# erererq/gym-lorenz

Hardware: NVIDIA B200
Metric: env_steps_per_sec (higher is better)
Workload: dtype f64

## Files before the change

### gym_lorenz_b200/csrc/chaos_b200.cu

```cuda
#include <math.h>
#include <pthread.h>
#include <sched.h>
#include <stdarg.h>
#include <time.h>
#include <stdio.h>
#include <stdlib.h>
#include <string.h>

#include "kernels_common.cuh"
#include "host_copy.h"

cudaError_t cl_launch_derivatives(int kind, const void* state, const float* action, void* out,
                                  int64_t n, cudaStream_t st);

using cl::KParams;

struct CopyHelper;

namespace {

const cl_layout kLayouts[CL_ENV_KIND_COUNT] = {
     {8, 4, 0, 6, 3, 0, -500.0, 500.0, -HUGE_VAL, HUGE_VAL, 0, 0},
     {8, 10, 0, 6, 3, 0, -500.0, 500.0, -HUGE_VAL, HUGE_VAL, 0, 0},
     {8, 9, 0, 8, 3, 0, -2.0, 2.0, -HUGE_VAL, HUGE_VAL, 0, 0},
// ... 355 lines not shown
  const double eff = (double)W / (double)(((W + nsched - 1) / nsched) * nsched);
  return eff < 0.95;
}

extern "C" int cl_rollout(cl_ctx* ctx, void* stream, const cl_buffers* buf, const cl_io* io,
                          const cl_rollout_desc* d) {
  if (!ctx) return fail(nullptr, CL_EINVAL, "null ctx");
  if (!io || !d || d->T < 1) return fail(ctx, CL_EINVAL, "cl_rollout: io/desc required, T >= 1");
  if (io->noise) return fail(ctx, CL_EINVAL, "cl_rollout: noise override is single-step only");
  KParams p;
  int r = fill_params(ctx, buf, io, p);
  if (r) return r;
  p.T = d->T; p.act_ts = d->act_ts; p.obs_ts = d->obs_ts; p.rew_ts = d->rew_ts; p.done_ts = d->done_ts;
  p.synth_amp = (float)d->synth_amp;
  cudaStream_t st = (cudaStream_t)stream;
  CU(cudaSetDevice(ctx->cfg.device));
  int chunk = CL_DYN_CHUNK_DEFAULT;
  if (const char* ov = getenv("CHAOS_B200_DYN_CHUNK")) { const int c = atoi(ov); if (c >= 1 && c <= 16) chunk = c; }
  int mode = cl::MODE_ROLLOUT;
  alignas(64) CUtensorMap tmap;
  if (want_dynamic(ctx, d->T, chunk)) {
    const int64_t W = (ctx->cfg.num_envs + 31) / 32;
    if (!ctx->dyn_bps) {
      int occ = 0;
      cudaError_t e = is_parity(ctx->cfg.kind) ? cl_dyn_occupancy_parity(ctx->cfg.kind, chunk, &occ)
                                               : cl_dyn_occupancy_northstar(ctx->cfg.kind, chunk, &occ);
      if (e != cudaSuccess) return fail(ctx, CL_ECUDA, "dyn occupancy query: %s", cudaGetErrorString(e));
      int bps = (int)(W / ((int64_t)ctx->sm_count * 4));
      bps = bps < 1 ? 1 : (bps > 4 ? 4 : bps);
      if (const char* ov = getenv("CHAOS_B200_DYN_BPS")) { const int b = atoi(ov); if (b >= 1 && b <= 16) bps = b; }
      ctx->dyn_bps = occ < bps ? occ : bps;
    }
    if (ctx->dyn_bps >= 1) {
      CU(cudaMemsetAsync(ctx->d_dyn, 0, sizeof(uint32_t) * (size_t)(W + 1), st));
      p.dyn_counter = ctx->d_dyn;
      p.dyn_progress = ctx->d_dyn + 1;
      p.dyn_chunk = chunk;
      p.dyn_nchunks = (d->T + chunk - 1) / chunk;
      p.dyn_nwarps = (int32_t)W;
      const int64_t workers = (int64_t)ctx->sm_count * ctx->dyn_bps;
      const int64_t tasks = W * (int64_t)((d->T + chunk - 1) / chunk);
      p.dyn_grid = (int32_t)(workers * 4 < tasks ? workers : (tasks + 3) / 4);
      p.dyn_tma = (io->action != nullptr && io->act_es == 1 && (io->act_cs % 4) == 0 && (d->act_ts % 4) == 0 &&
                   ((uintptr_t)io->action % 16) == 0 && io->act_cs >= W * 32) ? 1 : 0;
      {
        const char* ov = getenv("CHAOS_B200_SM");
        if (!(ov && ov[0] == '0') && p.dyn_tma) {
          const int grid = (int)(W < ctx->sm_count ? W : ctx->sm_count);
          const int qn = (int)(W / grid), cmax = (int)((W + grid - 1) / grid);
          int workers = qn >= 4 ? 4 * (qn / 4) : qn;
          workers = workers > 16 ? 16 : workers;
          if (workers == 16 && qn < 20) workers = 12;
          if (const char* w = getenv("CHAOS_B200_SM_WORKERS")) { const int k = atoi(w); if (k >= 1 && k <= 16) workers = k < qn ? k : qn; }
          int sc = 16;
          const size_t per_warp = (size_t)ctx->lay.n_state * 32u * (size_t)ctx->lay.real_bytes + 32u * 12u + 28u;
          while (sc > 1 && (size_t)cmax * (2u * (size_t)sc * (size_t)ctx->lay.act_dim * 128u + per_warp) + 256u > 200u * 1024u) sc /= 2;
          if (const char* w = getenv("CHAOS_B200_SM_CHUNK")) { const int k = atoi(w); if (k >= 1 && k <= 16) sc = k; }
          if (sc > d->T) sc = d->T;
          if (cmax <= 64) {
            p.sm_grid = grid; p.sm_workers = workers; p.sm_chunk = sc;
            p.sm_gdiv = 1;
            if (const char* w = getenv("CHAOS_B200_SM_GDIV")) { const int k = atoi(w); if (k >= 1 && k <= 16) p.sm_gdiv = k; }
            p.host_tmap = &tmap;
            p.sm_tmap_ok = action_tensor_map(&tmap, io->action, (uint64_t)W * 32, (uint64_t)ctx->lay.act_dim,
                                             (uint64_t)d->T, (uint64_t)io->act_cs, (uint64_t)d->act_ts, (uint32_t)sc) ? 1 : 0;
            const char* tm = getenv("CHAOS_B200_SM_TMAP");
            if (tm && tm[0] == '0') p.sm_tmap_ok = 0;
// ... 495 lines not shown
```

### gym_lorenz_b200/csrc/envs_northstar.cuh

```cuda
#pragma once
#include "kernels_common.cuh"

namespace cl {

template <typename R>
struct LorenzPar { R sigma, rho, beta; };

template <typename R>
__device__ __forceinline__ void lorenz_rhs_u(const LorenzPar<R>& q, R x, R y, R z, R u1, R u2, R u3,
                                             R& dx, R& dy, R& dz) {
  dx = fma(q.sigma, y - x, u1);
  dy = fma(x, q.rho - z, u2 - y);
  dz = fma(x, y, fma(-q.beta, z, u3));
}

template <typename R>
__device__ __forceinline__ void lorenz_rhs_s(const R sigma, const R beta, R x, R y, R zs, R u1, R u2, R c3,
                                             R& dx, R& dy, R& dz) {
  dx = fma(sigma, y - x, u1);
  dy = fma(-x, zs, u2 - y);
  dz = fma(x, y, fma(-beta, zs, c3));
}

#define CL_LORENZ_RK4_SUBSTEP()                                                                     \
  {                                                                                                 \
    R k1x, k1y, k1z, kx, ky, kz, ax, ay, az;                                                        \
    lorenz_rhs_s(sigma, beta, x, y, zs, u1, u2, c3, k1x, k1y, k1z);                                 \
    ax = fma(h6, k1x, x); ay = fma(h6, k1y, y); az = fma(h6, k1z, zs);                              \
    lorenz_rhs_s(sigma, beta, fma(hh, k1x, x), fma(hh, k1y, y), fma(hh, k1z, zs), u1, u2, c3, kx, ky, kz);   \
    ax = fma(h3, kx, ax); ay = fma(h3, ky, ay); az = fma(h3, kz, az);                               \
    lorenz_rhs_s(sigma, beta, fma(hh, kx, x), fma(hh, ky, y), fma(hh, kz, zs), u1, u2, c3, k1x, k1y, k1z);   \
    ax = fma(h3, k1x, ax); ay = fma(h3, k1y, ay); az = fma(h3, k1z, az);                            \
    lorenz_rhs_s(sigma, beta, fma(h, k1x, x), fma(h, k1y, y), fma(h, k1z, zs), u1, u2, c3, kx, ky, kz);      \
    x = fma(h6, kx, ax); y = fma(h6, ky, ay); zs = fma(h6, kz, az);                                 \
  }

template <typename R>
__device__ __forceinline__ void lorenz_rk4(const R sigma, const R rho, const R beta, const R br, R& x, R& y, R& z,
                                           R u1, R u2, R u3, const R h, const R hh, const R h3, const R h6,
                                           int substeps) {
  R zs = z - rho;
  const R c3 = u3 - br;
#pragma unroll 2
  for (int k = 0; k < substeps; ++k) CL_LORENZ_RK4_SUBSTEP()
  z = zs + rho;
}

template <typename R, int S>
__device__ __forceinline__ void lorenz_rk4_fixed(const R sigma, const R rho, const R beta, const R br, R& x, R& y,
                                                 R& z, R u1, R u2, R u3, const R h, const R hh, const R h3,
                                                 const R h6) {
  R zs = z - rho;
  const R c3 = u3 - br;
#pragma unroll
  for (int k = 0; k < S; ++k) CL_LORENZ_RK4_SUBSTEP()
  z = zs + rho;
}

template <typename R>
__device__ __forceinline__ void lorenz_rk4_any(const R sigma, const R rho, const R beta, const R br, R& x, R& y,
                                               R& z, R u1, R u2, R u3, const R h, const R hh, const R h3,
                                               const R h6, int S) {
  if (S == 16) {
    lorenz_rk4_fixed<R, 16>(sigma, rho, beta, br, x, y, z, u1, u2, u3, h, hh, h3, h6);
    return;
  }
  switch (S) {
    case 8: lorenz_rk4_fixed<R, 8>(sigma, rho, beta, br, x, y, z, u1, u2, u3, h, hh, h3, h6); break;
    case 4: lorenz_rk4_fixed<R, 4>(sigma, rho, beta, br, x, y, z, u1, u2, u3, h, hh, h3, h6); break;
    case 1: lorenz_rk4_fixed<R, 1>(sigma, rho, beta, br, x, y, z, u1, u2, u3, h, hh, h3, h6); break;
    default: lorenz_rk4<R>(sigma, rho, beta, br, x, y, z, u1, u2, u3, h, hh, h3, h6, S); break;
  }
}

template <typename R>
struct EnvLorenzRK4 {
  typedef R real;
  enum { NSTATE = 6, NINT = 0, OBS = 6, ACT = 3, NOISE = 0 };
  struct S { R x, y, z; LorenzPar<R> q; bool uni; };
  __device__ static void load(S& s, const KParams& p, int64_t i) {
    s.x = ldp<R>(p, 0, i); s.y = ldp<R>(p, 1, i); s.z = ldp<R>(p, 2, i);
    s.q.sigma = ldp<R>(p, 3, i); s.q.rho = ldp<R>(p, 4, i); s.q.beta = ldp<R>(p, 5, i);
  }
  __device__ static void prepare(S& s, const KParams& p, bool live) {
    const bool same = !live || (sizeof(R) == 8
        ? (s.q.sigma == (R)p.nom[0] && s.q.rho == (R)p.nom[1] && s.q.beta == (R)p.nom[2])
        : (s.q.sigma == (R)p.nomf[0] && s.q.rho == (R)p.nomf[1] && s.q.beta == (R)p.nomf[2]));
    s.uni = __all_sync(0xffffffffu, same);
  }
// ... 3 lines not shown
  }
  __device__ static void load_sm(S& s, const R* b, unsigned lane) {
    s.x = b[lane]; s.y = b[32 + lane]; s.z = b[64 + lane];
    s.q.sigma = b[96 + lane]; s.q.rho = b[128 + lane]; s.q.beta = b[160 + lane];
  }
  __device__ static void store_sm(const S& s, R* b, unsigned lane) {
    b[lane] = s.x; b[32 + lane] = s.y; b[64 + lane] = s.z;
  }
  __device__ static bool uses_noise(const KParams&) { return false; }
  __device__ static bool finite(const S& s) { return isfinite(s.x + s.y + s.z); }
  __device__ static bool time_limit(const KParams& p, int32_t n) {
    return p.max_steps > 0 && n >= p.max_steps;
  }
  __device__ static void init_persistent(S& s, const KParams& p, const Stream& rng) {
    double j[3] = {1.0, 1.0, 1.0};
    if (p.param_jitter > 0.0) draw_uniform<3>(rng, TAG_PARAM, 1.0 - p.param_jitter, 1.0 + p.param_jitter, j);
    s.q.sigma = (R)(10.0 * j[0]); s.q.rho = (R)(28.0 * j[1]); s.q.beta = (R)((8.0 / 3.0) * j[2]);
    s.x = s.y = s.z = R(0);
  }
  __device__ static void observe(const S& s, R* obs) {
    obs[0] = s.x; obs[1] = s.y; obs[2] = s.z;
    lorenz_rhs_u(s.q, s.x, s.y, s.z, R(0), R(0), R(0), obs[3], obs[4], obs[5]);
  }
  __device__ static void reset(S& s, const KParams&, const Stream& rng, R* obs) {
    double u[3];
    draw_uniform<3>(rng, TAG_RESET, -30.0, 30.0, u);
    s.x = (R)u[0]; s.y = (R)u[1]; s.z = (R)u[2];
    observe(s, obs);
  }
  __device__ static int spec(const S& s, const KParams& p) {
    return (s.uni && p.substeps == 16) ? 1 : 0;
  }
  template <int SPEC>
  __device__ static void step_spec(S& s, const KParams& p, const float* a, const double*, R* obs, R& rew,
                                   bool& term) {
    static_assert(SPEC == 1, "unknown specialisation");
    const float lim = p.act_limit_f;
    const R g = sizeof(R) == 8 ? (R)p.act_gain : (R)p.act_gain_f;
    const R u1 = mul_keep((R)clipf(a[0], -lim, lim), g);
    const R u2 = mul_keep((R)clipf(a[1], -lim, lim), g);
    const R u3 = mul_keep((R)clipf(a[2], -lim, lim), g);
    if (sizeof(R) == 8) {
      lorenz_rk4_fixed<R, 16>((R)p.nom[0], (R)p.nom[1], (R)p.nom[2], (R)p.nom_br, s.x, s.y, s.z, u1, u2, u3,
                              (R)p.h, (R)p.hh, (R)p.h3, (R)p.h6);
    } else {
      lorenz_rk4_fixed<R, 16>((R)p.nomf[0], (R)p.nomf[1], (R)p.nomf[2], (R)p.nom_brf, s.x, s.y, s.z, u1, u2, u3,
                              (R)p.hf, (R)p.hhf, (R)p.h3f, (R)p.h6f);
    }
    observe(s, obs);
    const R e = fabs(s.x) + fabs(s.y) + fabs(s.z);
    rew = -e;
    term = !(e <= R(1e6));
  }
  __device__ static void step(S& s, const KParams& p, const float* a, const double*, R* obs, R& rew,
                              bool& term) {
    const float lim = p.act_limit_f;
    const R g = sizeof(R) == 8 ? (R)p.act_gain : (R)p.act_gain_f;
    const R u1 = mul_keep((R)clipf(a[0], -lim, lim), g);
    const R u2 = mul_keep((R)clipf(a[1], -lim, lim), g);
    const R u3 = mul_keep((R)clipf(a[2], -lim, lim), g);
    if (s.uni) {
      if (sizeof(R) == 8)
        lorenz_rk4_any<R>((R)p.nom[0], (R)p.nom[1], (R)p.nom[2], (R)p.nom_br, s.x, s.y, s.z, u1, u2, u3,
                          (R)p.h, (R)p.hh, (R)p.h3, (R)p.h6, p.substeps);
      else
        lorenz_rk4_any<R>((R)p.nomf[0], (R)p.nomf[1], (R)p.nomf[2], (R)p.nom_brf, s.x, s.y, s.z, u1, u2, u3,
                          (R)p.hf, (R)p.hhf, (R)p.h3f, (R)p.h6f, p.substeps);
    } else {
      const R br = mul_rn(s.q.beta, s.q.rho);
      if (sizeof(R) == 8)
        lorenz_rk4_any<R>(s.q.sigma, s.q.rho, s.q.beta, br, s.x, s.y, s.z, u1, u2, u3,
                          (R)p.h, (R)p.hh, (R)p.h3, (R)p.h6, p.substeps);
      else
        lorenz_rk4_any<R>(s.q.sigma, s.q.rho, s.q.beta, br, s.x, s.y, s.z, u1, u2, u3,
                          (R)p.hf, (R)p.hhf, (R)p.h3f, (R)p.h6f, p.substeps);
    }
    observe(s, obs);
    const R e = fabs(s.x) + fabs(s.y) + fabs(s.z);
    rew = -e;
    term = !(e <= R(1e6));
  }
};

struct PMSMPar { double sigma, gamma; };

__device__ __forceinline__ void pmsm_rhs_u(const PMSMPar& q, const double* x, double u1, double u2,
                                           double* d) {
  d[0] = fma(x[1], x[2], u1 - x[0]);
  d[1] = fma(q.gamma - x[0], x[2], u2 - x[1]);
  d[2] = q.sigma * (x[1] - x[2]);
}

__device__ __forceinline__ void pmsm_rhs_s(const double sigma, const double* x, double c1, double u2, double* d) {
  d[0] = fma(x[1], x[2], c1 - x[0]);
  d[1] = fma(-x[0], x[2], u2 - x[1]);
  d[2] = sigma * (x[1] - x[2]);
}

#define CL_PMSM_RK4_SUBSTEP(x, c1, u2)                                                                    \
  {                                                                                                        \
    double k1[3], k2[3], w[3], acc[3];                                                                     \
    pmsm_rhs_s(sigma, x, c1, u2, k1);                                                                      \
    _Pragma("unroll") for (int c = 0; c < 3; ++c) { acc[c] = fma(h6, k1[c], x[c]); w[c] = fma(hh, k1[c], x[c]); }   \
    pmsm_rhs_s(sigma, w, c1, u2, k2);                                                                      \
    _Pragma("unroll") for (int c = 0; c < 3; ++c) { acc[c] = fma(h3, k2[c], acc[c]); w[c] = fma(hh, k2[c], x[c]); } \
    pmsm_rhs_s(sigma, w, c1, u2, k1);                                                                      \
    _Pragma("unroll") for (int c = 0; c < 3; ++c) { acc[c] = fma(h3, k1[c], acc[c]); w[c] = fma(h, k1[c], x[c]); }  \
    pmsm_rhs_s(sigma, w, c1, u2, k2);                                                                      \
    _Pragma("unroll") for (int c = 0; c < 3; ++c) x[c] = fma(h6, k2[c], acc[c]);                           \
  }

template <int S>
__device__ __forceinline__ void pmsm_rk4_pair(const double sigma, const double gamma, double* a, double* b,
// ... 93 lines not shown
                                   double& rew, bool& term) {
    static_assert(SPEC == 1, "unknown specialisation");
    const float lim = (float)p.act_limit;
    const double u1 = mul_keep((double)clipf(a[0], -lim, lim), p.act_gain);
    const double u2 = mul_keep((double)clipf(a[1], -lim, lim), p.act_gain);
    pmsm_rk4_pair_any(p.nom[0], p.nom[1], s.a, s.b, u1, u2, p.h, p.hh, p.h3, p.h6, p.substeps);
    finish(s, p, obs, rew, term);
  }
  __device__ static void finish(const S& s, const KParams& p, double* obs, double& rew, bool& term) {
    observe(s, obs);
    const double e0 = fabs(obs[0]), e1 = fabs(obs[1]), e2 = fabs(obs[2]);
    const double E = e0 + e1 + e2;
    rew = -E - (pow_pos(e0 + 1e-6, p.alpha) + pow_pos(e1 + 1e-6, p.alpha) + pow_pos(e2 + 1e-6, p.alpha));
    term = false;
    if (!(E <= 1000.0)) { rew = -1000.0; term = true; }
  }
  __device__ static void step(S& s, const KParams& p, const float* a, const double*, double* obs,
                              double& rew, bool& term) {
    const float lim = (float)p.act_limit;
    const double u1 = mul_keep((double)clipf(a[0], -lim, lim), p.act_gain);
    const double u2 = mul_keep((double)clipf(a[1], -lim, lim), p.act_gain);
    if (s.uni) pmsm_rk4_pair_any(p.nom[0], p.nom[1], s.a, s.b, u1, u2, p.h, p.hh, p.h3, p.h6, p.substeps);
    else pmsm_rk4_pair_any(s.q.sigma, s.q.gamma, s.a, s.b, u1, u2, p.h, p.hh, p.h3, p.h6, p.substeps);
    finish(s, p, obs, rew, term);
  }
};

template <> struct PlainRollout<EnvLorenzRK4<double>> { enum { value = 1 }; };
template <> struct PlainRollout<EnvLorenzRK4<float>> { enum { value = 1 }; };
template <> struct PlainRollout<EnvPMSMRK4> { enum { value = 1 }; };
template <> struct FiniteUnlessTerm<EnvLorenzRK4<double>> { enum { value = 1 }; };
template <> struct FiniteUnlessTerm<EnvLorenzRK4<float>> { enum { value = 1 }; };
template <> struct FiniteUnlessTerm<EnvPMSMRK4> { enum { value = 1 }; };

}
```

### gym_lorenz_b200/csrc/kernels_common.cuh

```cuda
#pragma once
#include <cuda.h>
#include <cuda_runtime.h>
#include <stdint.h>
#include <string.h>

#include "../../include/chaos_b200.h"
#include "philox.cuh"

namespace cl {

struct KParams {
  int64_t n, n_pad, env_id_base;
  int64_t i_begin;
  uint32_t k0, k1;
  uint64_t step_index;
  uint64_t* step_ptr;
  int32_t max_steps, substeps, flags, reward_f32;
  double dt, alpha, act_limit, act_gain, param_jitter;
  void* state;
  int32_t* aux_int;
  int32_t* ep_len;
  double* ep_return;
  double* stats;
  const float* action;
// ... 131 lines not shown
                                                    const int64_t warp_env0, const int64_t n, const unsigned lane,
                                                    const real* obs) {
#pragma unroll
  for (int c = 0; c < OBS; ++c) sm[lane * OBS + c] = (float)obs[c];
  __syncwarp();
  const int64_t rows = n - warp_env0;
  const int nflt = (int)(rows >= 32 ? 32 : (rows > 0 ? rows : 0)) * OBS;
  float* dst = base + warp_env0 * OBS;
  for (int k = (int)lane * 4; k + 3 < nflt; k += 128)
    *reinterpret_cast<float4*>(dst + k) = *reinterpret_cast<const float4*>(sm + k);
  for (int k = (nflt & ~3) + (int)lane; k < nflt; k += 32) dst[k] = sm[k];
  __syncwarp();
}

template <typename real>
__device__ __forceinline__ real ldp(const KParams& p, int c, int64_t i) {
  return __ldcg((const real*)p.state + (int64_t)c * p.n_pad + i);
}
template <typename real>
__device__ __forceinline__ void stp(const KParams& p, int c, int64_t i, real v) {
  ((real*)p.state)[(int64_t)c * p.n_pad + i] = v;
}

__device__ __forceinline__ uint32_t ld_acquire_sys_u32(const uint32_t* p) {
  uint32_t v;
  asm volatile("ld.acquire.sys.global.u32 %0, [%1];" : "=r"(v) : "l"(p) : "memory");
  return v;
}


template <class E> struct PlainRollout { enum { value = 0 }; };
template <class E> struct FiniteUnlessTerm { enum { value = 0 }; };
template <int N> struct SpecTag { enum { value = N }; };

#ifndef CL_PLAIN_DEFER
#define CL_PLAIN_DEFER 1
#endif
template <class E> struct PlainPending {
  typename E::real obs[E::OBS];
  typename E::real rew;
  uint32_t dflags, valid;
  int t;
  float* o;
  typename E::real* rp;
  uint8_t* dp;
  __device__ __forceinline__ void begin(const KParams& p, const int64_t i, const int t0) {
    const int64_t np = p.n_pad, row = (int64_t)t0 * np + i;
    o = (float*)p.obs + (int64_t)t0 * (E::OBS * np) + i;
    rp = (typename E::real*)p.reward + row;
    dp = p.done + row;
    t = t0;
    valid = 0u; dflags = 0u; rew = 0;
#pragma unroll
    for (int c = 0; c < E::OBS; ++c) obs[c] = 0;
  }
};
__device__ __forceinline__ void st_if(float* ptr, float v, uint32_t pr) {
  asm volatile("{\n.reg .pred p;\nsetp.ne.u32 p, %0, 0;\n@p st.global.f32 [%1], %2;\n}" ::"r"(pr), "l"(ptr), "f"(v) : "memory");
}
__device__ __forceinline__ void st_if(double* ptr, double v, uint32_t pr) {
  asm volatile("{\n.reg .pred p;\nsetp.ne.u32 p, %0, 0;\n@p st.global.f64 [%1], %2;\n}" ::"r"(pr), "l"(ptr), "d"(v) : "memory");
}
__device__ __forceinline__ void st_if(uint8_t* ptr, uint32_t v, uint32_t pr) {
  asm volatile("{\n.reg .pred p;\nsetp.ne.u32 p, %0, 0;\n@p st.global.u8 [%1], %2;\n}" ::"r"(pr), "l"(ptr), "r"(v) : "memory");
}
template <class E, bool RUNPTR>
// ... 5 lines not shown
#pragma unroll
    for (int c = 0; c < E::OBS; ++c) st_if(d.o + c * np, (float)d.obs[c], pr);
    st_if(d.rp, d.rew, pr);
    st_if(d.dp, d.dflags, pr);
    if (d.valid) {
      d.o += E::OBS * np;
      d.rp += np;
      d.dp += np;
    }
  } else {
    const int64_t row = (int64_t)d.t * np + i;
    float* o = (float*)p.obs + (int64_t)d.t * (E::OBS * np) + i;
#pragma unroll
    for (int c = 0; c < E::OBS; ++c) st_if(o + c * np, (float)d.obs[c], pr);
    st_if((real*)p.reward + row, d.rew, pr);
    st_if(p.done + row, d.dflags, pr);
  }
}

template <class E, int SPEC>
__device__ __forceinline__ void step_dispatch(typename E::S& s, const KParams& p, const float* a, const double* nz,
                                              typename E::real* obs, typename E::real& rew, bool& term) {
  if constexpr (SPEC != 0) E::template step_spec<SPEC>(s, p, a, nz, obs, rew, term);
  else E::step(s, p, a, nz, obs, rew, term);
}

template <class E>
struct TermOut {
  typename E::real obs[E::OBS];
  typename E::real rew;
  uint32_t dflags;
};

template <class E, bool ROLL, bool PLAIN = false, int SPEC = 0, bool RUNPTR = false, class TermPtr = decltype(nullptr)>
__device__ __forceinline__ unsigned env_interval(typename E::S& s, int32_t& ep_len, double& ep_ret,
                                             const KParams& p, const int64_t i, const bool live,
                                             const unsigned lane, const int t, const uint64_t step,
                                             const float* a, const bool want_noise, const bool obs64,
                                             const bool autoreset, unsigned& bad_acc, float* sm_rows, bool& fin,
                                             PlainPending<E>* pend = nullptr, double* blk_stats = nullptr,
                                             typename E::real* obs_out = nullptr, TermPtr term_out = nullptr) {
  typedef typename E::real real;
  if (PLAIN && CL_PLAIN_DEFER) plain_emit<E, RUNPTR>(p, i, live, *pend);
  Stream rng = {};
  if (!PLAIN) rng = make_stream(p, i, step);
  double nz[E::NOISE > 0 ? E::NOISE : 1];
  nz[0] = 0.0;
  if (want_noise) {
    if (p.noise != nullptr) {
#pragma unroll
      for (int c = 0; c < E::NOISE; ++c) nz[c] = live ? p.noise[c * p.n_pad + i] : 0.0;
    } else {
      draw_normal<(E::NOISE > 0 ? E::NOISE : 1)>(rng, TAG_NOISE, nz);
    }
  }

  real obs[E::OBS];
  real rew;
  bool term;
  const bool was_finite = fin;
  step_dispatch<E, SPEC>(s, p, a, nz, obs, rew, term);
  ep_len += 1;
  ep_ret += (double)rew;
  const bool trunc = E::time_limit(p, ep_len);
  const bool done = term || trunc;
  bool bad;
  if constexpr (PLAIN && FiniteUnlessTerm<E>::value != 0) {
    fin = true;
    bad = false;
    if (term) { fin = E::finite(s); bad = was_finite && !fin; }
  } else {
    fin = E::finite(s);
    bad = was_finite && !fin;
  }

  const bool has_term = !PLAIN && p.term_obs != nullptr;
  const unsigned dall = __ballot_sync(0xffffffffu, live && done && (autoreset || has_term));
  const unsigned dm = autoreset ? dall : 0u;
  const unsigned bm = __ballot_sync(0xffffffffu, live && bad);
  if (dm) {
    const bool mine = (dm >> lane) & 1u;
    const double r1 = warp_sum(mine ? ep_ret : 0.0);
    const double r2 = warp_sum(mine ? ep_ret * ep_ret : 0.0);
    const int l1 = warp_sum(mine ? ep_len : 0);
    const unsigned tm = __ballot_sync(0xffffffffu, mine && term);
    const unsigned um = __ballot_sync(0xffffffffu, mine && trunc && !term);
    if (lane == 0) {
      double* dst = blk_stats != nullptr ? blk_stats : p.stats;
      atomicAdd(&dst[CL_STAT_EPISODES], (double)__popc(dm));
      atomicAdd(&dst[CL_STAT_RET_SUM], r1);
      atomicAdd(&dst[CL_STAT_RET_SQ], r2);
      atomicAdd(&dst[CL_STAT_LEN_SUM], (double)l1);
      if (tm) atomicAdd(&dst[CL_STAT_TERMINATED], (double)__popc(tm));
      if (um) atomicAdd(&dst[CL_STAT_TRUNCATED], (double)__popc(um));
// ... 401 lines not shown
    }
    q = grab();
  }
}



template <class E>
struct SmLayout {
  typedef typename E::real real;
  size_t act, state, ep_ret, ep_len, mbar, prog, total;
  __host__ __device__ SmLayout(int cnt, int chunk) {
    size_t o = 0;
    act = o;    o += (size_t)cnt * 2 * chunk * E::ACT * 32 * sizeof(float);
    state = o;  o += (size_t)cnt * E::NSTATE * 32 * sizeof(real);
    ep_ret = o; o += (size_t)cnt * 32 * sizeof(double);
    ep_len = o; o += (size_t)cnt * 32 * sizeof(int32_t);
    mbar = o;   o += (size_t)cnt * 3 * sizeof(uint64_t);
    prog = o;   o += ((size_t)cnt + 1) * sizeof(uint32_t);
    total = (o + 127) & ~(size_t)127;
  }
};

__device__ __forceinline__ void tma_load_3d(void* dst, const void* tmap, int x, int y, int z, uint64_t* bar) {
  asm volatile(
      "cp.async.bulk.tensor.3d.shared::cluster.global.tile.mbarrier::complete_tx::bytes [%0], [%1, {%2, %3, %4}], [%5];"
      ::"r"(smem_u32(dst)), "l"(tmap), "r"(x), "r"(y), "r"(z), "r"(smem_u32(bar))
      : "memory");
}

#ifndef CL_SM_THREADS
#define CL_SM_THREADS 576
#endif
#ifndef CL_SM_MINB
#define CL_SM_MINB 0
#endif
template <class E>
__global__ void __launch_bounds__(CL_SM_THREADS, CL_SM_MINB) k_rollout_sm(const KParams p,
                                                                         const __grid_constant__ CUtensorMap tmap) {
  typedef typename E::real real;
  extern __shared__ __align__(128) unsigned char sm_raw[];
  const unsigned lane = threadIdx.x & 31u;
  const int wib = threadIdx.x >> 5, nres = blockDim.x >> 5;
  const int W = p.dyn_nwarps, G = (int)gridDim.x, b = (int)blockIdx.x;
  const int qn = W / G, rn = W % G;
  const int e0 = b * qn + (b < rn ? b : rn);
  const int cnt = qn + (b < rn ? 1 : 0);
  const int cmax = qn + (rn ? 1 : 0);
  const int ng = cnt - nres;
  const int Tc = p.sm_chunk, Tg = max(1, Tc / max(1, p.sm_gdiv));
  const int nchunks = 1 + (p.T - 1 + Tc - 1) / Tc;
  const int nchunks_g = 1 + (p.T - 1 + Tg - 1) / Tg;
  auto chunk_t0 = [&](int f, int c, int tc) { return c == 0 ? 0 : min(p.T, f + (c - 1) * tc); };
  auto chunk_len = [&](int f, int c, int tc) { return min(c == 0 ? f : tc, p.T - chunk_t0(f, c, tc)); };
  const SmLayout<E> L(cmax, Tc);
  float* const act = (float*)(sm_raw + L.act);
  real* const st = (real*)(sm_raw + L.state);
  double* const s_ret = (double*)(sm_raw + L.ep_ret);
  int32_t* const s_len = (int32_t*)(sm_raw + L.ep_len);
  uint64_t* const mbar = (uint64_t*)(sm_raw + L.mbar);
  volatile uint32_t* const prog = (volatile uint32_t*)(sm_raw + L.prog);
  uint32_t* const counter = (uint32_t*)(sm_raw + L.prog) + cmax;
  const int per_buf = Tc * E::ACT * 32;

  for (int k = threadIdx.x; k < cnt * 3; k += blockDim.x) mbar_init(&mbar[k], 1);
  for (int k = threadIdx.x; k <= cmax; k += blockDim.x) ((uint32_t*)(sm_raw + L.prog))[k] = 0u;
  for (int k = threadIdx.x; k < cnt * 32; k += blockDim.x) {
    const int le = k >> 5, ln = k & 31;
    const int64_t i = (int64_t)(e0 + le) * 32 + ln;
#pragma unroll
    for (int c = 0; c < E::NSTATE; ++c) st[(le * E::NSTATE + c) * 32 + ln] = ldp<real>(p, c, i);
    s_ret[k] = __ldcg(p.ep_return + i);
    s_len[k] = __ldcg(p.ep_len + i);
// ... 1 lines not shown
  asm volatile("fence.mbarrier_init.release.cluster;" ::: "memory");
  __syncthreads();

  auto stage = [&](int le, int f, int c, int tc) {
    const int t0 = chunk_t0(f, c, tc);
    uint64_t* bar = &mbar[le * 3 + (c & 1)];
    float* dst = act + (size_t)(le * 2 + (c & 1)) * per_buf;
    if (p.sm_tmap_ok) {
      if (lane == 0) {
        mbar_expect_tx(bar, (uint32_t)(per_buf * sizeof(float)));
        tma_load_3d(dst, &tmap, (e0 + le) * 32, 0, t0, bar);
      }
    } else {
      const int len = chunk_len(f, c, tc);
      if (lane == 0) mbar_expect_tx(bar, (uint32_t)(len * E::ACT * 128));
      __syncwarp();
      for (int k = (int)lane; k < len * E::ACT; k += 32) {
        const int tl = k / E::ACT, cc = k % E::ACT;
        const float* src = p.action + (int64_t)(t0 + tl) * p.act_ts + (int64_t)cc * p.act_cs + (int64_t)(e0 + le) * 32;
        bulk_g2s(dst + (tl * E::ACT + cc) * 32, src, 128u, bar);
      }
    }
  };
  auto wait_actions = [&](int le, int c) {
    uint64_t* bar = &mbar[le * 3 + (c & 1)];
    const uint32_t parity = (uint32_t)(c >> 1) & 1u;
    uint32_t spins = 0;
    while (!mbar_try_wait(bar, parity)) spin_guard(spins);
  };
  for (int le = wib; le < cnt; le += nres) { const int tc = le < nres ? Tc : Tg; stage(le, 1 + le * tc / cnt, 0, tc); }

  const uint64_t step0 = step_base(p);
  unsigned bad_acc = 0u;

  auto run_chunk = [&](typename E::S& s, int32_t& ep_len, double& ep_ret, bool& fin, PlainPending<E>& pend,
                       const int le, const int c, const int t0, const int len, const int64_t i, const bool live) {
    const float* ab = act + (size_t)(le * 2 + (c & 1)) * per_buf;
    auto intervals = [&](auto spec_tag) {
      constexpr int SPEC = decltype(spec_tag)::value;
      for (int tl = 0; tl < len; ++tl) {
        const int t = t0 + tl;
        const uint64_t step = step0 + (uint64_t)t;
        float a[E::ACT];
#pragma unroll
        for (int cc = 0; cc < E::ACT; ++cc) a[cc] = ab[(tl * E::ACT + cc) * 32 + lane];
        env_interval<E, true, true, SPEC, true>(s, ep_len, ep_ret, p, i, live, lane, t, step, a, false, false, true,
                                                bad_acc, nullptr, fin, &pend);
      }
    };
    if (E::spec(s, p) == 1) intervals(SpecTag<1>{});
    else intervals(SpecTag<0>{});
  };

  const uint32_t g_total = (uint32_t)ng * (uint32_t)nchunks_g;
  const int g_credit = ng * (Tc / Tg);
  typename E::S s = {};
  int32_t ep_len = 0;
  double ep_ret = 0.0;
  bool fin = true;
  PlainPending<E> pend;
  pend.valid = 0u;
  int in_regs = -1;
  int c_own = 0;
  int credit = (wib * g_credit) % nres;
  bool guests_left = ng > 0, want_guest = false;
  for (;;) {
    int le, c;
    bool guest;
    if (want_guest) {
      uint32_t q = 0;
      if (lane == 0) q = atomicAdd(counter, 1u);
      q = __shfl_sync(0xffffffffu, q, 0);
      if (q >= g_total) { guests_left = false; want_guest = false; continue; }
      guest = true; le = nres + (int)(q % (uint32_t)ng); c = (int)(q / (uint32_t)ng);
    } else if (c_own < nchunks) {
      guest = false; le = wib; c = c_own;
    } else if (guests_left) {
      want_guest = true;
      continue;
    } else {
      break;
    }
    const int tc = guest ? Tg : Tc, nch = guest ? nchunks_g : nchunks;
    const int f = 1 + le * tc / cnt;
    const int t0 = chunk_t0(f, c, tc), len = chunk_len(f, c, tc);
    const int64_t i = (int64_t)(e0 + le) * 32 + lane;
    const bool live = i < p.n;
    if (guest && c > 0) {
      uint32_t spins = 0;
      if (lane == 0) {
        while (prog[le] != (uint32_t)c) { __nanosleep(32); spin_guard(spins); }
      }
      __syncwarp();
      uint64_t* hb = &mbar[le * 3 + 2];
      const uint32_t parity = (uint32_t)(c - 1) & 1u;
      while (!mbar_try_wait(hb, parity)) spin_guard(spins);
    }
    if (c + 1 < nch) stage(le, f, c + 1, tc);
    if (in_regs != le) {
      E::load_sm(s, st + (size_t)le * E::NSTATE * 32, lane);
      ep_len = s_len[le * 32 + lane];
      ep_ret = s_ret[le * 32 + lane];
      E::prepare(s, p, live);
      fin = E::finite(s);
      pend.begin(p, i, t0);
      in_regs = le;
    }
    wait_actions(le, c);
    run_chunk(s, ep_len, ep_ret, fin, pend, le, c, t0, len, i, live);
    bool park;
    if (guest) {
      park = true;
      want_guest = false;
    } else {
      c_own += 1;
      credit += g_credit;
      want_guest = guests_left && credit >= nres && c_own < nchunks;
      if (want_guest) credit -= nres;
      park = want_guest || c_own == nchunks;
    }
    if (park) {
      E::store_sm(s, st + (size_t)le * E::NSTATE * 32, lane);
      s_len[le * 32 + lane] = ep_len;
      s_ret[le * 32 + lane] = ep_ret;
      if (guest) {
        __syncwarp();
        if (lane == 0) {
          prog[le] = (uint32_t)c + 1u;
          mbar_arrive(&mbar[le * 3 + 2]);
        }
      }
      if (CL_PLAIN_DEFER) plain_emit<E, true>(p, i, live, pend);
      pend.valid = 0u;
      in_regs = -1;
    }
  }
  if (bad_acc && lane == 0) atomicAdd(&p.stats[CL_STAT_NONFINITE], (double)bad_acc);

  __syncthreads();
  for (int k = threadIdx.x; k < cnt * 32; k += blockDim.x) {
    const int le = k >> 5, ln = k & 31;
    const int64_t i = (int64_t)(e0 + le) * 32 + ln;
    if (i < p.n) {
#pragma unroll
      for (int c = 0; c < E::NSTATE; ++c) stp<real>(p, c, i, st[(le * E::NSTATE + c) * 32 + ln]);
      p.ep_return[i] = s_ret[k];
      p.ep_len[i] = s_len[k];
    }
  }
}

template <class E>
__global__ void __launch_bounds__(256) k_reset(const KParams p) {
  typedef typename E::real real;
  const int64_t i = (int64_t)blockIdx.x * blockDim.x + threadIdx.x;
  const uint64_t step0 = step_base(p);
  if (i < p.n && (p.mask == nullptr || p.mask[i] != 0)) {
    typename E::S s = {};
    E::load(s, p, i);
    const Stream rng = make_stream(p, i, step0);
    real obs[E::OBS];
    E::reset(s, p, rng, obs);
    E::store(s, p, i);
    p.ep_len[i] = 0;
    p.ep_return[i] = 0.0;
    if (p.obs) store_obs<real>(p.obs, 0, p.obs_es, p.obs_cs, i, obs, E::OBS, (p.flags & CL_F_OBS_F64) != 0);
  }
}

template <class E>
__global__ void __launch_bounds__(256) k_init(const KParams p) {
  const int64_t i = (int64_t)blockIdx.x * blockDim.x + threadIdx.x;
// ... 35 lines not shown
  const unsigned grid = (unsigned)((p.n - p.i_begin + block - 1) / block);
  const unsigned step_grid = grid + ((mode == MODE_STEP && p.act_host_words != nullptr) ? 1u : 0u);
  switch (mode) {
    case MODE_STEP: k_step<E, false><<<step_grid, block, row_smem, st>>>(p); break;
    case MODE_ROLLOUT:
      if (plain) k_step<E, true, HAS_PLAIN><<<grid, block, row_smem, st>>>(p);
      else k_step<E, true><<<grid, block, row_smem, st>>>(p);
      break;
    case MODE_RESET: k_reset<E><<<grid, block, 0, st>>>(p); break;
    case MODE_INIT: k_init<E><<<grid, block, 0, st>>>(p); break;
    case MODE_ROLLOUT_DYN: {
      if constexpr (HAS_PLAIN) {
        if (plain && p.sm_grid > 0) {
          const int cmax = (p.dyn_nwarps + p.sm_grid - 1) / p.sm_grid;
          size_t smem = SmLayout<E>(cmax, p.sm_chunk).total;
          if (smem < 120 * 1024) smem = 120 * 1024;
          if (smem <= 200 * 1024) {
            static bool attr_set = false;
            if (!attr_set) {
              cudaError_t e = cudaFuncSetAttribute(k_rollout_sm<E>, cudaFuncAttributeMaxDynamicSharedMemorySize, 200 * 1024);
              if (e != cudaSuccess) return e;
              attr_set = true;
            }
            if (p_in.host_plain_out) *p_in.host_plain_out |= 2;
            alignas(64) CUtensorMap tm;
            if (p.sm_tmap_ok && p.host_tmap) tm = *p.host_tmap;
            else { memset(&tm, 0, sizeof(tm)); p.sm_tmap_ok = 0; }
            p.host_tmap = nullptr;
            k_rollout_sm<E><<<(unsigned)p.sm_grid, (unsigned)p.sm_workers * 32, smem, st>>>(p, tm);
            break;
          }
        }
      }
      const size_t smem = (size_t)4 * p.dyn_chunk * E::ACT * 32 * sizeof(float) + 4 * sizeof(uint64_t);
      if (plain) k_rollout_dyn<E, HAS_PLAIN><<<(unsigned)p.dyn_grid, 128, smem, st>>>(p);
      else k_rollout_dyn<E><<<(unsigned)p.dyn_grid, 128, smem, st>>>(p);
      break;
    }
    default: return cudaErrorInvalidValue;
  }
  return cudaGetLastError();
}

template <class E>
cudaError_t dyn_occupancy(int chunk, int* blocks_per_sm) {
  const size_t smem = (size_t)4 * chunk * E::ACT * 32 * sizeof(float) + 4 * sizeof(uint64_t);
  cudaError_t e = cudaFuncSetAttribute(k_rollout_dyn<E>, cudaFuncAttributePreferredSharedMemoryCarveout, 50);
  if (e != cudaSuccess) return e;
  int occ = 0, occ_plain = 1 << 30;
  e = cudaOccupancyMaxActiveBlocksPerMultiprocessor(&occ, k_rollout_dyn<E>, 128, smem);
  if (e != cudaSuccess) return e;
  if (PlainRollout<E>::value) {
    e = cudaFuncSetAttribute(k_rollout_dyn<E, PlainRollout<E>::value != 0>, cudaFuncAttributePreferredSharedMemoryCarveout, 50);
    if (e != cudaSuccess) return e;
    e = cudaOccupancyMaxActiveBlocksPerMultiprocessor(&occ_plain, k_rollout_dyn<E, PlainRollout<E>::value != 0>, 128, smem);
    if (e != cudaSuccess) return e;
  }
  *blocks_per_sm = occ < occ_plain ? occ : occ_plain;
  return cudaSuccess;
}

}

cudaError_t cl_launch_parity(int kind, const cl::KParams& p, int mode, cudaStream_t st, int block);
cudaError_t cl_launch_northstar(int kind, const cl::KParams& p, int mode, cudaStream_t st, int block);
cudaError_t cl_occupancy_parity(int kind, int block, int* blocks_per_sm);
// ... 9 lines not shown
```

### gym_lorenz_b200/csrc/tu_northstar.cu

```cuda
#include "envs_northstar.cuh"

using namespace cl;

#define CL_NS_KINDS(X)                              \
  X(CL_ENV_LORENZ_RK4, EnvLorenzRK4<double>)        \
  X(CL_ENV_LORENZ_RK4_F32, EnvLorenzRK4<float>)     \
  X(CL_ENV_PMSM_RK4, EnvPMSMRK4)

cudaError_t cl_launch_northstar(int kind, const KParams& p, int mode, cudaStream_t st, int block) {
  switch (kind) {
#define X(K, E) case K: return launch_env<E>(p, mode, st, block);
    CL_NS_KINDS(X)
#undef X
    default: return cudaErrorInvalidValue;
  }
}

cudaError_t cl_occupancy_northstar(int kind, int block, int* out) {
  switch (kind) {
#define X(K, E) case K: return cudaOccupancyMaxActiveBlocksPerMultiprocessor(out, k_step<E, true>, block, 0);
    CL_NS_KINDS(X)
#undef X
    default: return cudaErrorInvalidValue;
  }
}

cudaError_t cl_dyn_occupancy_northstar(int kind, int chunk, int* out) {
  switch (kind) {
#define X(K, E) case K: return dyn_occupancy<E>(chunk, out);
    CL_NS_KINDS(X)
#undef X
    default: return cudaErrorInvalidValue;
  }
}

template <typename R>
__global__ void __launch_bounds__(256) k_fma_peak(int iters, R* sink) {
  R a[8];
  const R m = R(1.0) - R(1e-7), c = R(1e-9);
#pragma unroll
  for (int j = 0; j < 8; ++j) a[j] = R(threadIdx.x + j) * R(1e-3);
  for (int it = 0; it < iters; ++it) {
#pragma unroll
    for (int r = 0; r < 16; ++r) {
#pragma unroll
      for (int j = 0; j < 8; ++j) a[j] = fma(a[j], m, c);
    }
  }
  R s = R(0);
#pragma unroll
  for (int j = 0; j < 8; ++j) s += a[j];
  if (s == R(-1.2345)) sink[0] = s;
}

cudaError_t cl_fma_peak_launch(int dtype_bytes, int grid, int block, int iters, void* sink, cudaStream_t st) {
  if (dtype_bytes == 8) k_fma_peak<double><<<grid, block, 0, st>>>(iters, (double*)sink);
  else k_fma_peak<float><<<grid, block, 0, st>>>(iters, (float*)sink);
  return cudaGetLastError();
}
```

Before: 21.76 billion.

## Software-pipeline Lorenz action decode one step ahead in SM rollout kernel

Splits the Lorenz step into control (clip, scale and fold the nominal beta*rho term into c3) and advance, and in the shared-memory rollout kernel computes the next step's control while the current RK4 integration runs, using an empty asm barrier to pin the precomputed values in registers. The goal is to take action load and decode latency off the dependent RK4 chain. It also moves the dyn-counter memset into the dyn launch branch so it only runs when the dyn kernel launches, and adds compile-time optional globaltimer instrumentation. This adds register pressure and a somewhat more complex per-step control flow.

Result: no change. 21.88 billion, median of 6 (+0.6%).

```diff
diff --git a/gym_lorenz_b200/csrc/chaos_b200.cu b/gym_lorenz_b200/csrc/chaos_b200.cu
--- a/gym_lorenz_b200/csrc/chaos_b200.cu
+++ b/gym_lorenz_b200/csrc/chaos_b200.cu
@@ -411,7 +411,6 @@
       ctx->dyn_bps = occ < bps ? occ : bps;
     }
     if (ctx->dyn_bps >= 1) {
-      CU(cudaMemsetAsync(ctx->d_dyn, 0, sizeof(uint32_t) * (size_t)(W + 1), st));
       p.dyn_counter = ctx->d_dyn;
       p.dyn_progress = ctx->d_dyn + 1;
       p.dyn_chunk = chunk;
diff --git a/gym_lorenz_b200/csrc/envs_northstar.cuh b/gym_lorenz_b200/csrc/envs_northstar.cuh
--- a/gym_lorenz_b200/csrc/envs_northstar.cuh
+++ b/gym_lorenz_b200/csrc/envs_northstar.cuh
@@ -47,14 +47,19 @@
 }
 
 template <typename R, int S>
+__device__ __forceinline__ void lorenz_rk4_fixed_c3(const R sigma, const R rho, const R beta, R& x, R& y, R& z,
+                                                    R u1, R u2, const R c3, const R h, const R hh, const R h3,
+                                                    const R h6) {
+  R zs = z - rho;
+#pragma unroll
+  for (int k = 0; k < S; ++k) CL_LORENZ_RK4_SUBSTEP()
+  z = zs + rho;
+}
+template <typename R, int S>
 __device__ __forceinline__ void lorenz_rk4_fixed(const R sigma, const R rho, const R beta, const R br, R& x, R& y,
                                                  R& z, R u1, R u2, R u3, const R h, const R hh, const R h3,
                                                  const R h6) {
-  R zs = z - rho;
-  const R c3 = u3 - br;
-#pragma unroll
-  for (int k = 0; k < S; ++k) CL_LORENZ_RK4_SUBSTEP()
-  z = zs + rho;
+  lorenz_rk4_fixed_c3<R, S>(sigma, rho, beta, x, y, z, u1, u2, u3 - br, h, hh, h3, h6);
 }
 
 template <typename R>
@@ -124,34 +129,21 @@
     return (s.uni && p.substeps == 16) ? 1 : 0;
   }
   template <int SPEC>
-  __device__ static void step_spec(S& s, const KParams& p, const float* a, const double*, R* obs, R& rew,
-                                   bool& term) {
-    static_assert(SPEC == 1, "unknown specialisation");
+  __device__ static void integrate(S& s, const KParams& p, const float* a) {
     const float lim = p.act_limit_f;
     const R g = sizeof(R) == 8 ? (R)p.act_gain : (R)p.act_gain_f;
     const R u1 = mul_keep((R)clipf(a[0], -lim, lim), g);
     const R u2 = mul_keep((R)clipf(a[1], -lim, lim), g);
     const R u3 = mul_keep((R)clipf(a[2], -lim, lim), g);
-    if (sizeof(R) == 8) {
-      lorenz_rk4_fixed<R, 16>((R)p.nom[0], (R)p.nom[1], (R)p.nom[2], (R)p.nom_br, s.x, s.y, s.z, u1, u2, u3,
-                              (R)p.h, (R)p.hh, (R)p.h3, (R)p.h6);
-    } else {
-      lorenz_rk4_fixed<R, 16>((R)p.nomf[0], (R)p.nomf[1], (R)p.nomf[2], (R)p.nom_brf, s.x, s.y, s.z, u1, u2, u3,
-                              (R)p.hf, (R)p.hhf, (R)p.h3f, (R)p.h6f);
-    }
-    observe(s, obs);
-    const R e = fabs(s.x) + fabs(s.y) + fabs(s.z);
-    rew = -e;
-    term = !(e <= R(1e6));
-  }
-  __device__ static void step(S& s, const KParams& p, const float* a, const double*, R* obs, R& rew,
-                              bool& term) {
-    const float lim = p.act_limit_f;
-    const R g = sizeof(R) == 8 ? (R)p.act_gain : (R)p.act_gain_f;
-    const R u1 = mul_keep((R)clipf(a[0], -lim, lim), g);
-    const R u2 = mul_keep((R)clipf(a[1], -lim, lim), g);
-    const R u3 = mul_keep((R)clipf(a[2], -lim, lim), g);
-    if (s.uni) {
+    if (SPEC == 1) {
+      if (sizeof(R) == 8) {
+        lorenz_rk4_fixed<R, 16>((R)p.nom[0], (R)p.nom[1], (R)p.nom[2], (R)p.nom_br, s.x, s.y, s.z, u1, u2, u3,
+                                (R)p.h, (R)p.hh, (R)p.h3, (R)p.h6);
+      } else {
+        lorenz_rk4_fixed<R, 16>((R)p.nomf[0], (R)p.nomf[1], (R)p.nomf[2], (R)p.nom_brf, s.x, s.y, s.z, u1, u2, u3,
+                                (R)p.hf, (R)p.hhf, (R)p.h3f, (R)p.h6f);
+      }
+    } else if (s.uni) {
       if (sizeof(R) == 8)
         lorenz_rk4_any<R>((R)p.nom[0], (R)p.nom[1], (R)p.nom[2], (R)p.nom_br, s.x, s.y, s.z, u1, u2, u3,
                           (R)p.h, (R)p.hh, (R)p.h3, (R)p.h6, p.substeps);
@@ -167,10 +159,51 @@
         lorenz_rk4_any<R>(s.q.sigma, s.q.rho, s.q.beta, br, s.x, s.y, s.z, u1, u2, u3,
                           (R)p.hf, (R)p.hhf, (R)p.h3f, (R)p.h6f, p.substeps);
     }
-    observe(s, obs);
+  }
+  __device__ static void judge(const S& s, R& rew, bool& term) {
     const R e = fabs(s.x) + fabs(s.y) + fabs(s.z);
     rew = -e;
     term = !(e <= R(1e6));
+  }
+  template <int SPEC>
+  __device__ static void step_spec(S& s, const KParams& p, const float* a, const double*, R* obs, R& rew,
+                                   bool& term) {
+    static_assert(SPEC == 1, "unknown specialisation");
+    integrate<1>(s, p, a);
+    observe(s, obs);
+    judge(s, rew, term);
+  }
+  __device__ static void step(S& s, const KParams& p, const float* a, const double*, R* obs, R& rew,
+                              bool& term) {
+    integrate<0>(s, p, a);
+    observe(s, obs);
+    judge(s, rew, term);
+  }
+  struct U { R u1, u2, c3; float a[3]; };
+  template <int SPEC>
+  __device__ static U control(const S&, const KParams& p, const float* a) {
+    U u;
+    if constexpr (SPEC == 1 && sizeof(R) == 8) {
+      const float lim = p.act_limit_f;
+      u.u1 = mul_keep((R)clipf(a[0], -lim, lim), (R)p.act_gain);
+      u.u2 = mul_keep((R)clipf(a[1], -lim, lim), (R)p.act_gain);
+      u.c3 = mul_keep((R)clipf(a[2], -lim, lim), (R)p.act_gain) - (R)p.nom_br;
+      asm volatile("" : "+d"(u.u1), "+d"(u.u2), "+d"(u.c3));
+    } else {
+#pragma unroll
+      for (int c = 0; c < 3; ++c) u.a[c] = a[c];
+    }
+    return u;
+  }
+  template <int SPEC>
+  __device__ static void advance(S& s, const KParams& p, const U& u, R* obs, R& rew, bool& term) {
+    if (SPEC == 1 && sizeof(R) == 8)
+      lorenz_rk4_fixed_c3<R, 16>((R)p.nom[0], (R)p.nom[1], (R)p.nom[2], s.x, s.y, s.z, u.u1, u.u2, u.c3,
+                                 (R)p.h, (R)p.hh, (R)p.h3, (R)p.h6);
+    else
+      integrate<SPEC>(s, p, u.a);
+    observe(s, obs);
+    judge(s, rew, term);
   }
 };
 
@@ -330,5 +363,7 @@
 template <> struct FiniteUnlessTerm<EnvLorenzRK4<double>> { enum { value = 1 }; };
 template <> struct FiniteUnlessTerm<EnvLorenzRK4<float>> { enum { value = 1 }; };
 template <> struct FiniteUnlessTerm<EnvPMSMRK4> { enum { value = 1 }; };
-
-}
+template <> struct IntervalPipeline<EnvLorenzRK4<double>> { enum { value = 1 }; };
+template <> struct IntervalPipeline<EnvLorenzRK4<float>> { enum { value = 1 }; };
+
+}
diff --git a/gym_lorenz_b200/csrc/kernels_common.cuh b/gym_lorenz_b200/csrc/kernels_common.cuh
--- a/gym_lorenz_b200/csrc/kernels_common.cuh
+++ b/gym_lorenz_b200/csrc/kernels_common.cuh
@@ -187,6 +187,7 @@
 template <class E> struct PlainRollout { enum { value = 0 }; };
 template <class E> struct FiniteUnlessTerm { enum { value = 0 }; };
 template <int N> struct SpecTag { enum { value = N }; };
+template <class E> struct IntervalPipeline { enum { value = 0 }; };
 
 #ifndef CL_PLAIN_DEFER
 #define CL_PLAIN_DEFER 1
@@ -258,15 +259,18 @@
   uint32_t dflags;
 };
 
-template <class E, bool ROLL, bool PLAIN = false, int SPEC = 0, bool RUNPTR = false, class TermPtr = decltype(nullptr)>
+template <class E, bool ROLL, bool PLAIN = false, int SPEC = 0, bool RUNPTR = false, class TermPtr = decltype(nullptr),
+          class CtlPtr = decltype(nullptr)>
 __device__ __forceinline__ unsigned env_interval(typename E::S& s, int32_t& ep_len, double& ep_ret,
                                              const KParams& p, const int64_t i, const bool live,
                                              const unsigned lane, const int t, const uint64_t step,
                                              const float* a, const bool want_noise, const bool obs64,
                                              const bool autoreset, unsigned& bad_acc, float* sm_rows, bool& fin,
                                              PlainPending<E>* pend = nullptr, double* blk_stats = nullptr,
-                                             typename E::real* obs_out = nullptr, TermPtr term_out = nullptr) {
+                                             typename E::real* obs_out = nullptr, TermPtr term_out = nullptr,
+                                             CtlPtr ctl = nullptr) {
   typedef typename E::real real;
+  constexpr bool PIPE = !std::is_same<CtlPtr, decltype(nullptr)>::value;
   if (PLAIN && CL_PLAIN_DEFER) plain_emit<E, RUNPTR>(p, i, live, *pend);
   Stream rng = {};
   if (!PLAIN) rng = make_stream(p, i, step);
@@ -285,7 +289,12 @@
   real rew;
   bool term;
   const bool was_finite = fin;
-  step_dispatch<E, SPEC>(s, p, a, nz, obs, rew, term);
+  if constexpr (PIPE) {
+    E::template advance<SPEC>(s, p, *ctl, obs, rew, term);
+    *ctl = E::template control<SPEC>(s, p, a);
+  } else {
+    step_dispatch<E, SPEC>(s, p, a, nz, obs, rew, term);
+  }
   ep_len += 1;
   ep_ret += (double)rew;
   const bool trunc = E::time_limit(p, ep_len);
@@ -753,6 +762,19 @@
 #ifndef CL_SM_THREADS
 #define CL_SM_THREADS 576
 #endif
+enum { CL_TL_START, CL_TL_OWN_END, CL_TL_GUEST_END, CL_TL_ARRIVE, CL_TL_LEAVE, CL_TL_SWITCH_NS, CL_TL_SWITCHES,
+       CL_TL_SMID, CL_TL_SLOTS, CL_TL_MAX_BLOCKS = 256 };
+#ifdef CL_SM_TIMELINE
+static __device__ unsigned long long cl_sm_timeline[CL_TL_MAX_BLOCKS * 16 * CL_TL_SLOTS];
+__device__ __forceinline__ unsigned long long tl_now() {
+  unsigned long long t;
+  asm volatile("mov.u64 %0, %%globaltimer;" : "=l"(t) :: "memory");
+  return t;
+}
+#define CL_TL(slot, v) do { if (lane == 0 && blockIdx.x < CL_TL_MAX_BLOCKS) cl_sm_timeline[(blockIdx.x * 16 + wib) * CL_TL_SLOTS + (slot)] = (v); } while (0)
+#else
+#define CL_TL(slot, v) do { } while (0)
+#endif
 #ifndef CL_SM_MINB
 #define CL_SM_MINB 0
 #endif
@@ -760,6 +782,7 @@
 __global__ void __launch_bounds__(CL_SM_THREADS, CL_SM_MINB) k_rollout_sm(const KParams p,
                                                                          const __grid_constant__ CUtensorMap tmap) {
   typedef typename E::real real;
+  constexpr bool PIPE = IntervalPipeline<E>::value != 0;
   extern __shared__ __align__(128) unsigned char sm_raw[];
   const unsigned lane = threadIdx.x & 31u;
   const int wib = threadIdx.x >> 5, nres = blockDim.x >> 5;
@@ -827,20 +850,45 @@
 
   const uint64_t step0 = step_base(p);
   unsigned bad_acc = 0u;
+#ifdef CL_SM_TIMELINE
+  unsigned long long tl_prev = tl_now(), tl_switch_ns = 0, tl_guest_end = 0;
+  uint32_t tl_switches = 0;
+  {
+    uint32_t smid;
+    asm volatile("mov.u32 %0, %%smid;" : "=r"(smid));
+    CL_TL(CL_TL_SMID, smid);
+    CL_TL(CL_TL_START, tl_prev);
+  }
+#endif
 
   auto run_chunk = [&](typename E::S& s, int32_t& ep_len, double& ep_ret, bool& fin, PlainPending<E>& pend,
                        const int le, const int c, const int t0, const int len, const int64_t i, const bool live) {
     const float* ab = act + (size_t)(le * 2 + (c & 1)) * per_buf;
     auto intervals = [&](auto spec_tag) {
       constexpr int SPEC = decltype(spec_tag)::value;
-      for (int tl = 0; tl < len; ++tl) {
-        const int t = t0 + tl;
-        const uint64_t step = step0 + (uint64_t)t;
+      if constexpr (PIPE) {
         float a[E::ACT];
 #pragma unroll
-        for (int cc = 0; cc < E::ACT; ++cc) a[cc] = ab[(tl * E::ACT + cc) * 32 + lane];
-        env_interval<E, true, true, SPEC, true>(s, ep_len, ep_ret, p, i, live, lane, t, step, a, false, false, true,
-                                                bad_acc, nullptr, fin, &pend);
+        for (int cc = 0; cc < E::ACT; ++cc) a[cc] = ab[cc * 32 + lane];
+        typename E::U ctl = E::template control<SPEC>(s, p, a);
+        for (int tl = 0; tl < len; ++tl) {
+          const int t = t0 + tl, tn = min(tl + 1, len - 1);
+          const uint64_t step = step0 + (uint64_t)t;
+#pragma unroll
+          for (int cc = 0; cc < E::ACT; ++cc) a[cc] = ab[(tn * E::ACT + cc) * 32 + lane];
+          env_interval<E, true, true, SPEC, true>(s, ep_len, ep_ret, p, i, live, lane, t, step, a, false, false, true,
+                                                  bad_acc, nullptr, fin, &pend, nullptr, nullptr, nullptr, &ctl);
+        }
+      } else {
+        for (int tl = 0; tl < len; ++tl) {
+          const int t = t0 + tl;
+          const uint64_t step = step0 + (uint64_t)t;
+          float a[E::ACT];
+#pragma unroll
+          for (int cc = 0; cc < E::ACT; ++cc) a[cc] = ab[(tl * E::ACT + cc) * 32 + lane];
+          env_interval<E, true, true, SPEC, true>(s, ep_len, ep_ret, p, i, live, lane, t, step, a, false, false, true,
+                                                  bad_acc, nullptr, fin, &pend);
+        }
       }
     };
     if (E::spec(s, p) == 1) intervals(SpecTag<1>{});
@@ -902,7 +950,17 @@
       in_regs = le;
     }
     wait_actions(le, c);
+#ifdef CL_SM_TIMELINE
+    const unsigned long long tl_run = tl_now();
+    tl_switch_ns += tl_run - tl_prev;
+    tl_switches += 1;
+#endif
     run_chunk(s, ep_len, ep_ret, fin, pend, le, c, t0, len, i, live);
+#ifdef CL_SM_TIMELINE
+    tl_prev = tl_now();
+    if (guest) tl_guest_end = tl_prev;
+    else if (c_own + 1 == nchunks) CL_TL(CL_TL_OWN_END, tl_prev);
+#endif
     bool park;
     if (guest) {
       park = true;
@@ -932,7 +990,16 @@
   }
   if (bad_acc && lane == 0) atomicAdd(&p.stats[CL_STAT_NONFINITE], (double)bad_acc);
 
+#ifdef CL_SM_TIMELINE
+  CL_TL(CL_TL_GUEST_END, tl_guest_end);
+  CL_TL(CL_TL_SWITCH_NS, tl_switch_ns);
+  CL_TL(CL_TL_SWITCHES, tl_switches);
+  CL_TL(CL_TL_ARRIVE, tl_now());
   __syncthreads();
+  CL_TL(CL_TL_LEAVE, tl_now());
+#else
+  __syncthreads();
+#endif
   for (int k = threadIdx.x; k < cnt * 32; k += blockDim.x) {
     const int le = k >> 5, ln = k & 31;
     const int64_t i = (int64_t)(e0 + le) * 32 + ln;
@@ -1034,6 +1101,10 @@
           }
         }
       }
+      {
+        const cudaError_t e = cudaMemsetAsync(p.dyn_counter, 0, sizeof(uint32_t) * ((size_t)p.dyn_nwarps + 1), st);
+        if (e != cudaSuccess) return e;
+      }
       const size_t smem = (size_t)4 * p.dyn_chunk * E::ACT * 32 * sizeof(float) + 4 * sizeof(uint64_t);
       if (plain) k_rollout_dyn<E, HAS_PLAIN><<<(unsigned)p.dyn_grid, 128, smem, st>>>(p);
       else k_rollout_dyn<E><<<(unsigned)p.dyn_grid, 128, smem, st>>>(p);
diff --git a/gym_lorenz_b200/csrc/tu_northstar.cu b/gym_lorenz_b200/csrc/tu_northstar.cu
--- a/gym_lorenz_b200/csrc/tu_northstar.cu
+++ b/gym_lorenz_b200/csrc/tu_northstar.cu
@@ -34,6 +34,13 @@
   }
 }
 
+#ifdef CL_SM_TIMELINE
+extern "C" int cl_sm_timeline_read(unsigned long long* dst, int slots_per_warp, int max_blocks) {
+  if (slots_per_warp != CL_TL_SLOTS || max_blocks != CL_TL_MAX_BLOCKS) return -1;
+  return cudaMemcpyFromSymbol(dst, cl_sm_timeline, sizeof(cl_sm_timeline)) == cudaSuccess ? 0 : -2;
+}
+#endif
+
 template <typename R>
 __global__ void __launch_bounds__(256) k_fma_peak(int iters, R* sink) {
   R a[8];
```
